# JOP-Lee/READ

Measured on AMD Instinct MI355X. Metric: rendered frames/sec @1216x352, 30M pts, higher is better.
Workload: dtype f32 (matrix-core products from two f16 pieces per operand, three piece pairs, fp32 accumulation)

## Files before the change

### read_amd/csrc/conv.hip

```cpp
#include <limits.h>

#include "common.h"
#include "internal.h"

using namespace readhip;

typedef float floatx16 __attribute__((ext_vector_type(16)));

namespace {

constexpr long long OOB_LIMIT = 0x7ffffff0ll;

struct SrcDev {
    const float *p;
    int C, H, W;
    int sl, sr;
};

struct ConvKArgs {
    SrcDev src[READ_CONV_MAX_SRC];
    const float *mul;
    const float *wp;
    const float *wp_wino;
    const float *wp_w16;
// ... 2341 lines not shown
#pragma unroll
            for (int px = 0; px < 4; ++px) {
                const bool in = (oy + 2 * py < a.outH) & (ox + px < a.outW) & (c0 < a.Cout);
                const int pix = (oy + 2 * py) * a.outW + ox + px;
                rvoff[px] = in ? (unsigned)((pix * a.Cout + c0) * 4) : OOR;
                ovoff[px] = in ? (unsigned)((pix * a.out_cstride + c0) * 4) : OOR;
            }
            f32x4 rv[4];
#pragma unroll
            for (int px = 0; px < 4; ++px) {
                rv[px] = f32x4{0.f, 0.f, 0.f, 0.f};
                if (a.residual) rv[px] = __builtin_bit_cast(f32x4, __builtin_amdgcn_raw_buffer_load_b128(res_rsrc, rvoff[px], 0, 0));
            }
            f32x4 Y[2][4];
#pragma unroll
            for (int h = 0; h < 2; ++h) {
                f32x4 m[6];
#pragma unroll
                for (int fq = 0; fq < 6; ++fq)
#pragma unroll
                    for (int k = 0; k < 4; ++k) asm volatile("v_accvgpr_read_b32 %0, %1" : "=v"(m[fq][k]) : "a"(acc[py + 2 * h][fq][k]));
                at6(m, Y[h]);
                __builtin_amdgcn_sched_barrier(0);
            }
#pragma unroll
            for (int px = 0; px < 4; ++px) {
                f32x4 yf, ym;
                fm_swap(Y[0][px], Y[1][px], yf, ym);
                f32x4 f = __builtin_elementwise_fma(yf, isf, bf);
                const f32x4 mm = __builtin_elementwise_fma(ym, ism, bml);
                if (a.elu) {
                    const f32x4 fe = f * LOG2E;
                    f32x4 e;
#pragma unroll
                    for (int k = 0; k < 4; ++k) e[k] = __builtin_amdgcn_exp2f(fe[k]);
                    e = e + f32x4{-1.0f, -1.0f, -1.0f, -1.0f};
#pragma unroll
                    for (int k = 0; k < 4; ++k) f[k] = f[k] > 0.0f ? f[k] : e[k];
                }
                f32x4 sg_, t;
#pragma unroll
                for (int k = 0; k < 4; ++k) t[k] = __builtin_amdgcn_exp2f(mm[k]);
                t = t + f32x4{1.0f, 1.0f, 1.0f, 1.0f};
#pragma unroll
                for (int k = 0; k < 4; ++k) sg_[k] = __builtin_amdgcn_rcpf(t[k]);
                const f32x4 v = (f * sg_) * sc + sh + rv[px];
                __builtin_amdgcn_raw_buffer_store_b128(__builtin_bit_cast(u32x4, v), out_rsrc, ovoff[px], 0, 0);
                __builtin_amdgcn_sched_barrier(0);
            }
        }
        step_tile(a, by, bx);
        advance();
        gload_patch();
    }
}

struct D3hGeom {
    static constexpr int IH = 10, IW = 34, NPIX = IH * IW;
    static constexpr int XBUF = NPIX * 32;
    static constexpr int NE = NPIX * 8, NI = (NE + 511) / 512;
};

template <bool MUL>
__global__ __launch_bounds__(512, 1) void gated_conv_d3h_kernel(const ConvKArgs a)
{
    using DG = D3hGeom;
    __shared__ __attribute__((aligned(16))) unsigned lds[2 * DG::XBUF];
    __shared__ __attribute__((aligned(16))) float epar[6][32];
    const int tid = threadIdx.x, lane = tid & 63;
    const int wv = __builtin_amdgcn_readfirstlane(tid >> 6), rh = wv & 1, pq = wv >> 1;
    const SrcDev s = a.src[0];
    const int groups = a.CoutPad >> 5, G = gridDim.x;
    const int g = blockIdx.x % groups;
    const int n = a.nchunks;
    constexpr unsigned OOR = 0x80000000u;

    int by = (blockIdx.x / groups) / a.tiles_x, bx = (blockIdx.x / groups) % a.tiles_x;
    int pby = by, pbx = bx, pu = blockIdx.x, pchunk = 0;

    int soff[DG::NI];
    unsigned rel[DG::NI], aoff[DG::NI];
#pragma unroll
    for (int i = 0; i < DG::NI; ++i) {
        const int e = tid + i * 512, pix = e >> 3, q4 = e & 7, ppx = pix % DG::IW;
        soff[i] = pix * 32 + ((((q4 >> 1)) ^ (ppx & 7)) << 2) + ((q4 & 1) << 1);
        rel[i] = (unsigned)(((pix / DG::IW) * s.W + ppx) * s.C + 4 * q4) * 4u;
    }
    const unsigned src_bytes = (unsigned)(a.inH * s.W * s.C) * 4u;
    const auto rsrc = __builtin_amdgcn_make_buffer_rsrc(const_cast<float *>(s.p), 0, src_bytes, 0x00020000);
    const auto rsrc_mul = __builtin_amdgcn_make_buffer_rsrc(const_cast<float *>(MUL ? a.mul : s.p), 0, src_bytes, 0x00020000);
    auto set_patch = [&]() {
        const int y0 = pby * 8 - 1, x0 = pbx * 32 - 1;
        const unsigned base = (unsigned)((y0 * s.W + x0) * s.C) * 4u;
#pragma unroll
        for (int i = 0; i < DG::NI; ++i) {
            const int e = tid + i * 512, pix = e >> 3, ppy = pix / DG::IW, ppx = pix % DG::IW;
            const bool ok = (e < DG::NE) & (ppy >= -y0) & (ppy < a.inH - y0) & (ppx >= -x0) & (ppx < a.inW - x0);
            aoff[i] = ok ? base + rel[i] : OOR;
        }
    };
    auto advance = [&]() {
        if (cursor_advance(a, n, G, pchunk, pu, pby, pbx)) set_patch();
    };
    float4 st[DG::NI], stm[MUL ? DG::NI : 1];
    auto gload = [&]() {
#pragma unroll
// ... 1017 lines not shown
    CFGNM(3, 1, 16, 2, 1, 2, 2, 2, 1),
    CFG(3, 1, 8, 2, 1, 4, 1, 2),
    CFG(3, 1, 8, 1, 1, 4, 1, 2),
    CFG(1, 1, 16, 2, 1, 4, 1, 1),
    CFG(1, 1, 16, 1, 1, 4, 1, 1),
    CFG(1, 1, 16, 2, 2, 2, 2, 1),
    CFG(1, 1, 32, 2, 1, 4, 1, 1),
    CFG(1, 1, 32, 1, 1, 4, 1, 1),
    CFG(1, 1, 32, 2, 2, 2, 2, 1),
    CFG(1, 1, 8, 2, 1, 4, 1, 0),
    CFG(1, 1, 8, 1, 1, 4, 1, 0),
    CFG(3, 2, 16, 1, 1, 4, 1, 1),
    CFG(3, 2, 16, 1, 2, 2, 2, 1),
    CFG(3, 2, 16, 1, 2, 4, 1, 1),
    CFGW(3, 1, 16, 2, 1, 1, 2),
    CFGW(3, 1, 16, 2, 1, 2, 2),
    CFGW(3, 1, 16, 1, 1, 2, 3),
    CFGW(1, 1, 16, 2, 1, 1, 2),
    CFGW(1, 1, 16, 1, 1, 1, 4),
    CFGW(1, 1, 32, 2, 1, 1, 2),
    CFGW(1, 1, 32, 1, 1, 1, 4),
    CFGW(3, 1, 8, 2, 1, 2, 2),
    {"k3s1c16_p1q1_wino", 3, 1, 16, 1, 1, 4, 1, 1, 2, gated_conv_wino_kernel<false, false>, gated_conv_wino_kernel<false, true>, 0, 0, 1},
    CFG(4, 2, 16, 1, 1, 1, 1, 1),
    CFG(4, 2, 16, 1, 1, 4, 1, 1),
    CFG(4, 2, 16, 1, 2, 2, 2, 1),
};
constexpr int N_CONFIGS = sizeof(g_configs) / sizeof(g_configs[0]);

int find_config(int ks, int s, int kc, int P, int QG, int WM, int WN, int PF, int NB)
{
    for (int i = 0; i < N_CONFIGS; ++i) {
        const ConvConfig &c = g_configs[i];
        if (c.KS == ks && c.S == s && c.KC == kc && c.P == P && c.QG == QG && c.WM == WM && c.WN == WN && c.PF == PF &&
            c.NB == NB)
            return i;
    }
    return -1;
}

enum ConvForce {
    CFG_AUTO = -1,
    CFG_PX = -2,
    CFG_W16 = -3,
    CFG_W4 = -5,
    CFG_SC = -6,
    CFG_W4H = -7,
    CFG_D3H = -8,
    CFG_D3H_S2 = -9,
    CFG_PXH = -10,
    CFG_T3H = -11,
    CFG_F4X1 = -12,
    CFG_F4X1_PAIR = -13,
};

int g_prefer_wave = 1;
int g_wino_wgs = 2;
int g_conv_px = 1;
int g_kc32 = 1;
int g_use_wino = 1 << 30;
int g_w4_grid = 0;
int g_w4 = 32;
int g_w4h = 32;
int g_f4x1 = 32;
int g_d3h = 0;
int g_d3h_fam = 32;
int g_d3h_s2 = 32;
int g_pxh = 16;
int g_t3h = 8;
int g_sc = 8;
int g_w16 = 0;
int g_stagger_ticks = 0;

int find_wave_config(int ks, int s, int kc, int P, int QG)
{
    int best = -1;
    for (int i = 0; i < N_CONFIGS; ++i) {
        const ConvConfig &c = g_configs[i];
        if (c.wave && c.KS == ks && c.S == s && c.KC == kc && c.P == P && c.QG == QG) best = i;
    }
    return best;
}

int first_fit(int ks, int s, int kc, int groups, bool tiled_only = false, bool with_mul = false)
{
    for (int i = 0; i < N_CONFIGS; ++i) {
        const ConvConfig &k = g_configs[i];
        if (k.KS == ks && k.S == s && k.KC == kc && groups % (k.WN * k.QG) == 0 && !(tiled_only && (k.wave || k.wino)) && !(with_mul && !k.fn_mul)) return i;
    }
    return -1;
}

int pick_config(int ks, int s, int kc, int groups, int outH, int outW)
{
    const long pixels = (long)outH * outW;
    int c = -1;
    if (ks == 3 && s == 1 && kc == 16) {
        if (groups % 4 == 0 && groups % 8 != 0) c = find_config(3, 1, 16, 2, 2, 2, 2, 1, 2);
        else if (g_prefer_wave) c = find_wave_config(3, 1, 16, 1, 1);
        else if (groups % 8 == 0) c = find_config(3, 1, 16, 2, 1, 2, 2, 2, 1);
        else c = find_config(3, 1, 16, 1, 1, 4, 1, 2, 1);
    } else if (ks == 3 && s == 1 && kc == 8) {
        c = (g_prefer_wave && pixels > 30000) ? find_wave_config(3, 1, 8, 2, 1) : find_config(3, 1, 8, 1, 1, 4, 1, 2, 2);
    } else if (ks == 1 && s == 1 && kc == 32) {
        const long wgs4 = (long)ceil_div(outW, 32) * ceil_div(outH, 4) * (groups / 4);
        if (groups % 4 == 0 && wgs4 >= 128) c = find_config(1, 1, 32, 2, 2, 2, 2, 1, 2);
// ... 64 lines not shown
    {"conv_w4h", &g_w4h, TN_CLAMP, 0, INT_MAX},
    {"conv_f4x1", &g_f4x1, TN_CLAMP, 0, INT_MAX},
    {"conv_d3h", &g_d3h, TN_CLAMP, 0, INT_MAX},
    {"conv_d3h_fam", &g_d3h_fam, TN_CLAMP, 0, INT_MAX},
    {"conv_d3h_s2", &g_d3h_s2, TN_CLAMP, 0, INT_MAX},
    {"conv_pxh", &g_pxh, TN_CLAMP, 0, INT_MAX},
    {"conv_t3h", &g_t3h, TN_CLAMP, 0, INT_MAX},
    {"conv_w4_grid", &g_w4_grid, TN_FLAG, 0, 0},
    {"conv_stagger", &g_stagger_ticks, TN_CLAMP, 0, INT_MAX},
    {"conv_wave", &g_prefer_wave, TN_FLAG, 0, 0},
};
constexpr int N_CONV_KNOBS = sizeof(g_knobs) / sizeof(g_knobs[0]);

int conv_set(const char *key, int v) { return tune_set(g_knobs, N_CONV_KNOBS, key, v); }
int conv_get(const char *key, int *value) { return tune_get(g_knobs, N_CONV_KNOBS, key, value); }
const char *conv_key(int i) { return tune_key(g_knobs, N_CONV_KNOBS, i); }

static unsigned long long *g_trace = nullptr;
static size_t g_trace_records = 0;
void conv_set_trace(void *buf, size_t bytes)
{
    g_trace = (unsigned long long *)buf;
    g_trace_records = buf ? bytes / 64 : 0;
}


static int conv_uses_wino(const read_conv_desc *d)
{
    return d->config < 0 && g_use_wino && !d->pre && d->ksize == 3 && d->stride == 1 && d->n_src == 1 &&
           d->src[0].shift == 0 && d->src[0].C % 16 == 0 && d->wpacked_wino && d->src[0].C <= g_use_wino;
}

static int conv_uses_w4(const read_conv_desc *d)
{
    const bool shape = !d->pre && (!d->linear || !d->residual) && d->ksize == 3 && d->stride == 1 && d->n_src == 1 && d->src[0].shift == 0 &&
                       d->src[0].C % 16 == 0 && d->src[0].C >= 32 && (d->Cout % 32 == 0 || (d->linear && d->Cout % 8 == 0)) && !d->fill_pad && d->wpacked_w4 &&
                       d->out_cstride % 4 == 0 &&
                       (long long)d->src[0].srcH * d->src[0].srcW * d->src[0].C * 4 < (1ll << 31) &&
                       (long long)d->inH * d->inW * d->out_cstride * 4 < (1ll << 31);
    return shape && (d->config == CFG_W4 || (d->config == CFG_AUTO && g_w4 > 0 && d->src[0].C >= g_w4));
}

static int conv_w4_shape(const read_conv_desc *d, const void *operand, bool with_threshold = false)
{
    read_conv_desc t = *d;
    if (!with_threshold) t.config = CFG_W4;
    t.wpacked_w4 = reinterpret_cast<const float *>(operand);
    return conv_uses_w4(&t);
}

static int conv_uses_w4h(const read_conv_desc *d)
{
    if (!d->wpacked_w4h || d->linear || d->mul || d->src[0].C % 32 != 0 || d->Cout % 32 != 0) return 0;
    const bool forced = d->config == CFG_W4H || d->config == CFG_F4X1 || d->config == CFG_F4X1_PAIR;
    if (!forced && (d->config != CFG_AUTO || g_w4h <= 0 || d->src[0].C < g_w4h)) return 0;
    return conv_w4_shape(d, d->wpacked_w4h, !forced);
}

static int conv_uses_d3h(const read_conv_desc *d)
{
    if (!d->wpacked_d3h || d->linear || d->src[0].C % 32 != 0 || d->Cout % 32 != 0) return 0;
    const int min_c = d->mul ? g_d3h_fam : g_d3h;
    if (!(d->config == CFG_D3H || (d->config == CFG_AUTO && min_c > 0 && d->src[0].C >= min_c))) return 0;
    return conv_w4_shape(d, d->wpacked_d3h);
}

static int conv_uses_d3h_s2(const read_conv_desc *d)
{
    const bool shape = d->wpacked_d3h && !d->linear && !d->mul && !d->pre && !d->fill_pad && (d->ksize == 3 || d->ksize == 4) && d->stride == 2 && d->n_src == 1 &&
                       d->src[0].shift == 0 && d->src[0].C % 32 == 0 && d->Cout % 32 == 0 && d->out_cstride % 4 == 0 &&
                       (long long)d->src[0].srcH * d->src[0].srcW * d->src[0].C * 4 < (1ll << 31) &&
                       (long long)d->inH * d->inW * d->out_cstride * 4 < (1ll << 31);
    return shape && (d->config == CFG_D3H_S2 || (d->config == CFG_AUTO && g_d3h_s2 > 0 && d->src[0].C >= g_d3h_s2));
}

static int conv_uses_pxh(const read_conv_desc *d)
{
    if (!d->wpacked_d3h || d->ksize != 1 || d->stride != 1 || d->mul || d->fill_pad || d->n_src < 1 || d->n_src > READ_CONV_MAX_SRC) return 0;
    if (d->pre && d->pre_bilinear) return 0;
    int Cin = 0;
    for (int i = 0; i < d->n_src; ++i) {
        if (d->src[i].C < 8 || d->src[i].C % 8 != 0 || (uintptr_t)d->src[i].data % 16 != 0) return 0;
        Cin += d->src[i].C;
    }
    const bool shape = Cin % 16 == 0 && Cin <= 256 && d->Cout % 4 == 0 && d->out_cstride % 4 == 0 && (uintptr_t)d->out % 16 == 0 &&
                       (uintptr_t)d->params % 16 == 0 && (!d->residual || (uintptr_t)d->residual % 16 == 0) &&
                       (!d->pre || ((uintptr_t)d->pre % 16 == 0 && d->pre_cstride % 4 == 0 && d->pre_f_off % 4 == 0 && d->pre_m_off % 4 == 0));
    return shape && (d->config == CFG_PXH || (d->config == CFG_AUTO && g_pxh > 0 && Cin >= g_pxh));
}

static int conv_uses_t3h(const read_conv_desc *d)
{
    if (!d->wpacked_t3h || d->ksize != 3 || d->stride != 1 || d->mul || d->fill_pad || d->pre || d->n_src != 1 || d->src[0].shift != 0) return 0;
    const int C = d->src[0].C;
    const bool shape = (C == 8 || C == 16 || C == 32) && d->Cout % 4 == 0 && d->out_cstride % 4 == 0 && (uintptr_t)d->out % 16 == 0 &&
                       (uintptr_t)d->src[0].data % 16 == 0 && (uintptr_t)d->params % 16 == 0 && (!d->residual || (uintptr_t)d->residual % 16 == 0) &&
                       (long long)d->inH * d->inW * C * 4 < (1ll << 31);
    return shape && (d->config == CFG_T3H || (d->config == CFG_AUTO && g_t3h > 0 && C <= g_t3h && (long long)d->inH * d->inW >= 16384));
}

static int conv_uses_sc(const read_conv_desc *d)
{
    const bool shape = d->ksize == 3 && d->stride == 1 && d->n_src == 1 && d->src[0].shift == 0 && d->src[0].C == 32 && d->Cout >= 1 &&
                       d->Cout <= 4 && !d->linear && !d->residual && !d->pre && !d->mul && d->wpacked_sc &&
                       (d->out_cstride != 4 || (uintptr_t)d->out % 16 == 0) &&
                       (long long)d->src[0].srcH * d->src[0].srcW * d->src[0].C * 4 < (1ll << 31);
    return shape && (d->config == CFG_SC || (d->config == CFG_AUTO && g_sc));
}

static bool conv_sane(const read_conv_desc *d)
{
    return d->n_src >= 1 && d->n_src <= READ_CONV_MAX_SRC && (d->ksize == 1 || d->ksize == 3 || d->ksize == 4) && (d->stride == 1 || d->stride == 2);
}

static int conv_uses_px(const read_conv_desc *d)
{
    if (!conv_sane(d)) return 0;
    int Cin = 0;
    bool px_pick = d->Cout % 32 != 0 || g_conv_px >= 3;
    for (int i = 0; i < d->n_src; ++i) {
        Cin += d->src[i].C;
        px_pick = px_pick || d->src[i].C % 16 != 0;
    }
    const bool fits = d->ksize == 1 && d->stride == 1 && !d->mul && !d->fill_pad && d->Cout % 4 == 0 && d->out_cstride % 4 == 0 &&
                      (uintptr_t)d->out % 16 == 0 && (uintptr_t)d->params % 16 == 0 && Cin / 8 <= 32 &&
                      (!d->residual || (uintptr_t)d->residual % 16 == 0) &&
                      (!d->pre || ((uintptr_t)d->pre % 16 == 0 && d->pre_cstride % 4 == 0 && d->pre_f_off % 4 == 0 && d->pre_m_off % 4 == 0));
    const bool bil = d->pre && d->pre_bilinear;
    return fits && (d->config == CFG_PX || (bil && d->config < 0) || (d->config == CFG_AUTO && g_conv_px && px_pick));
}

struct ConvShape {
    int Cin, kc;
    int outH, outW, CoutPad, groups;
};

static ConvShape conv_shape(const read_conv_desc *d)
{
    ConvShape s;
    s.Cin = 0;
    s.kc = 16;
    bool all32 = d->ksize == 1;
    for (int i = 0; i < d->n_src; ++i) {
        s.Cin += d->src[i].C;
        if (d->src[i].C % 16) s.kc = 8;
        all32 = all32 && d->src[i].C % 32 == 0;
    }
    if (all32 && (d->config >= 0 ? (d->config < N_CONFIGS && g_configs[d->config].KC == 32) : g_kc32 != 0)) s.kc = 32;
    const int pad = (d->ksize - 1) / 2;
    s.outH = (d->inH + 2 * pad - d->ksize) / d->stride + 1;
    s.outW = (d->inW + 2 * pad - d->ksize) / d->stride + 1;
    s.CoutPad = pad32(d->Cout);
    s.groups = s.CoutPad / 32;
    return s;
}

enum ConvKernel { CK_SC, CK_T3H, CK_PXH, CK_PX, CK_D3H_S2, CK_D3H, CK_F4X1, CK_F4X1_PAIR, CK_W4H, CK_W4, CK_TABLE };

struct ConvRoute {
    ConvKernel kernel;
    int cfg;
    bool wino_auto;
    bool w16;
};

static int w4_units(const ConvShape &s) { return ceil_div(s.outW, 32) * ceil_div(s.outH, 8) * s.groups; }

static bool f4x1_pair_auto(int Cin, int n_units, int n_cu) { return n_units > n_cu && (Cin == 32 || Cin == 128); }

static ConvRoute conv_route(const read_conv_desc *d, const void *wp_f4x1)
{
    ConvRoute r = {CK_TABLE, -1, false, false};
    if (conv_uses_sc(d)) r.kernel = CK_SC;
    else if (conv_uses_t3h(d)) r.kernel = CK_T3H;
    else if (conv_uses_pxh(d)) r.kernel = CK_PXH;
    else if (conv_uses_px(d)) r.kernel = CK_PX;
    else if (conv_uses_d3h_s2(d)) r.kernel = CK_D3H_S2;
    else if (conv_uses_d3h(d)) r.kernel = CK_D3H;
    else if (conv_uses_w4h(d)) {
        const bool forced = d->config == CFG_F4X1 || d->config == CFG_F4X1_PAIR;
        const bool f4x1 = wp_f4x1 && (forced || (d->config == CFG_AUTO && g_f4x1 > 0 && d->src[0].C >= g_f4x1));
        const bool pair = f4x1 && (d->config == CFG_F4X1_PAIR ||
                                   (d->config == CFG_AUTO && f4x1_pair_auto(d->src[0].C, w4_units(conv_shape(d)), device_cus())));
        r.kernel = !f4x1 ? CK_W4H : pair ? CK_F4X1_PAIR : CK_F4X1;
    }
    else if (conv_uses_w4(d)) r.kernel = CK_W4;
    else if (conv_sane(d)) {
        const ConvShape s = conv_shape(d);
        r.cfg = d->config;
        r.wino_auto = conv_uses_wino(d);
        for (int i = N_CONFIGS - 1; r.wino_auto && i >= 0; --i)
            if (g_configs[i].wino) r.cfg = i;
        if (d->linear && r.cfg < 0) r.cfg = first_fit(d->ksize, d->stride, s.kc, s.groups, true, d->mul != nullptr);
        if (r.cfg < 0) r.cfg = pick_config(d->ksize, d->stride, s.kc, s.groups, s.outH, s.outW);
        if (d->config < 0 && d->mul && r.cfg >= 0 && !g_configs[r.cfg].fn_mul) {
            const int m = first_fit(d->ksize, d->stride, s.kc, s.groups, false, true);
            if (m >= 0) r.cfg = m;
        }
        const bool mostly_padding = d->Cout <= 8;
        r.w16 = r.cfg >= 0 && r.cfg < N_CONFIGS && g_configs[r.cfg].wino && !d->linear && d->wpacked_w16 &&
                (d->config == CFG_W16 || (d->config < 0 && (g_w16 || mostly_padding)));
    }
    return r;
}

static int route_family(const ConvRoute &r)
{
    static const int family[] = { 1,  8,  7,  0,  6,  6,
                                  5,  5,  5,  4,  0};
    return r.wino_auto ? 2 : family[r.kernel];
}

int conv_family(const read_conv_desc *d) { return route_family(conv_route(d, nullptr)); }

static int conv_prepare(const read_conv_desc *d, const void *wp_f4x1, ConvKArgs &a, ConvShape &s, ConvRoute &r)
{
    READ_CHECK_ARG(d, "read_gated_conv_forward: null descriptor");
    READ_CHECK_ARG(d->n_src >= 1 && d->n_src <= READ_CONV_MAX_SRC, "read_gated_conv_forward: n_src must be 1..%d",
                   READ_CONV_MAX_SRC);
    READ_CHECK_ARG(d->ksize == 1 || d->ksize == 3 || d->ksize == 4, "read_gated_conv_forward: ksize must be 1,3,4");
    READ_CHECK_ARG(d->stride == 1 || d->stride == 2, "read_gated_conv_forward: stride must be 1 or 2");
    READ_CHECK_ARG(d->inH >= 1 && d->inW >= 1 && d->Cout >= 1, "read_gated_conv_forward: bad sizes");
    READ_CHECK_ARG((d->wpacked || d->wpacked_w4 || d->wpacked_w4h || d->wpacked_d3h || d->wpacked_wino || d->wpacked_t3h || wp_f4x1) && d->params && d->out, "read_gated_conv_forward: null weights/params/out");
    READ_CHECK_ARG(d->out_cstride >= (d->linear ? 2 : 1) * d->Cout, "read_gated_conv_forward: out_cstride too small");
    READ_CHECK_ARG(!d->linear || (!d->residual && !d->fill_pad), "read_gated_conv_forward: linear mode takes no residual / fill");
    READ_CHECK_ARG(!d->mul || d->n_src == 1, "read_gated_conv_forward: mul needs a single source");
    READ_CHECK_ARG((uintptr_t)d->wpacked % 16 == 0, "read_gated_conv_forward: packed weights misaligned");
    r = conv_route(d, wp_f4x1);
    s = conv_shape(d);
    {
        const int family = route_family(r);
        const bool cfg_wino = d->config >= 0 && d->config < N_CONFIGS && g_configs[d->config].wino;
        const bool w16_forced = d->config == CFG_W16;
        READ_CHECK_ARG(d->wpacked || family != 0 || cfg_wino || w16_forced,
                       "read_gated_conv_forward: this launch takes a direct kernel and wpacked is NULL (fragment order not packed)");
        READ_CHECK_ARG(!d->wpacked || (!((const void *)d->wpacked == (const void *)d->wpacked_w4 && family != 4 && family != 5 && family != 6 && family != 7 && family != 8) &&
                                       !((const void *)d->wpacked == (const void *)d->wpacked_wino && family != 2 && !cfg_wino)),
                       "read_gated_conv_forward: wpacked aliases Winograd fragments but the launch takes kernel family %d "
                       "(ask read_conv_kernel_family before packing)", family);
        READ_CHECK_ARG(family != 4 || d->wpacked_w4, "read_gated_conv_forward: F(4x4) launch without wpacked_w4");
        READ_CHECK_ARG(family != 2 || d->wpacked_wino, "read_gated_conv_forward: F(2x2) launch without wpacked_wino");
        READ_CHECK_ARG(family != 1 || d->wpacked_sc, "read_gated_conv_forward: small-Cout launch without wpacked_sc");
    }

    memset(&a, 0, sizeof(a));
    for (int i = 0; i < d->n_src; ++i) {
        const read_conv_src &src = d->src[i];
        READ_CHECK_ARG(src.data && (uintptr_t)src.data % 16 == 0, "read_gated_conv_forward: source %d null or misaligned", i);
        READ_CHECK_ARG(src.C >= 8 && src.C % 8 == 0, "read_gated_conv_forward: source %d has C=%d (need a multiple of 8)", i, src.C);
        READ_CHECK_ARG(src.shift >= -4 && src.shift <= 4, "read_gated_conv_forward: shift out of range");
        READ_CHECK_ARG((long long)src.srcH * src.srcW * src.C < (1ll << 31), "read_gated_conv_forward: source too large");
        const int needH = src.shift >= 0 ? ((d->inH - 1) << src.shift) + 1 : ((d->inH - 1) >> -src.shift) + 1;
        const int needW = src.shift >= 0 ? ((d->inW - 1) << src.shift) + 1 : ((d->inW - 1) >> -src.shift) + 1;
        READ_CHECK_ARG(src.srcH >= needH && src.srcW >= needW, "read_gated_conv_forward: source %d (%dx%d) too small for %dx%d at shift %d",
                       i, src.srcH, src.srcW, d->inH, d->inW, src.shift);
        a.src[i] = SrcDev{src.data, src.C, src.srcH, src.srcW, src.shift > 0 ? src.shift : 0, src.shift < 0 ? -src.shift : 0};
    }
    READ_CHECK_ARG(!d->mul || d->src[0].shift == 0, "read_gated_conv_forward: mul needs shift 0");
    a.n_src = d->n_src;
    READ_CHECK_ARG(s.outH >= 1 && s.outW >= 1, "read_gated_conv_forward: empty output");
    READ_CHECK_ARG((long long)s.outH * s.outW * d->out_cstride * 4 < OOB_LIMIT, "read_gated_conv_forward: output too large");
    if (d->pre) {
// ... 95 lines not shown
    a.nchunks = nsteps;
    a.n_units = ceil_div(s.outH * s.outW, 32 * pt);
    const bool fullq = nsteps % 4 == 0;
    bool uni = true;
    for (int i = 0; i < d->n_src; ++i) uni = uni && d->src[i].C % 16 == 0;
    const int shape = gw == 2 ? 0 : pt == 2 ? 1 : 2, vi = taps ? 12 + shape : shape * 4 + (fullq ? 2 : 0) + (uni ? 1 : 0);
    static const conv_fn fns[15] = {
        gated_conv_pxh_kernel<1, 2, false, 0>, gated_conv_pxh_kernel<1, 2, false, 1>, gated_conv_pxh_kernel<1, 2, true, 0>, gated_conv_pxh_kernel<1, 2, true, 1>,
        gated_conv_pxh_kernel<2, 1, false, 0>, gated_conv_pxh_kernel<2, 1, false, 1>, gated_conv_pxh_kernel<2, 1, true, 0>, gated_conv_pxh_kernel<2, 1, true, 1>,
        gated_conv_pxh_kernel<1, 1, false, 0>, gated_conv_pxh_kernel<1, 1, false, 1>, gated_conv_pxh_kernel<1, 1, true, 0>, gated_conv_pxh_kernel<1, 1, true, 1>,
        gated_conv_pxh_kernel<1, 2, false, 2>, gated_conv_pxh_kernel<2, 1, false, 2>, gated_conv_pxh_kernel<1, 1, false, 2>};
    static bool attr_set_h[15] = {false, false, false, false, false, false, false, false, false, false, false, false, false, false, false};
    return launch_pixel_lane(fns[vi], attr_set_h[vi], 80 * 1024, n_cu * per_cu, gsets, true, lds, stream, a);
}

static int launch_px(ConvKArgs &a, const ConvShape &s, hipStream_t stream)
{
    const int n_cu = device_cus(), nsteps = s.Cin / 8;
    const int gw = (s.groups % 2 == 0 && nsteps <= 16) ? 2 : 1;
    const bool wide = g_conv_px == 2 || g_conv_px == 4;
    const int pt = (gw == 2 ? 1 : 2) * (wide ? 2 : 1);
    const size_t lds = (size_t)nsteps * 2 * gw * 1024;
    int per_cu = (int)((160 * 1024) / (lds + 256));
    const int reg_cap = wide ? 2 : 3;
    per_cu = per_cu < 1 ? 1 : per_cu > reg_cap ? reg_cap : per_cu;
    const int gsets = s.groups / gw;
    a.nchunks = nsteps;
    a.n_units = ceil_div(s.outH * s.outW, 32 * pt);
    const bool fullq = nsteps % 4 == 0;
    static const conv_fn fns[8] = {gated_conv_px_kernel<2, 1>, gated_conv_px_kernel<4, 1>, gated_conv_px_kernel<1, 2>, gated_conv_px_kernel<2, 2>,
                                   gated_conv_px_kernel<2, 1, true>, gated_conv_px_kernel<4, 1, true>, gated_conv_px_kernel<1, 2, true>, gated_conv_px_kernel<2, 2, true>};
    static bool attr_set[8] = {false, false, false, false, false, false, false, false};
    const int vi = (gw == 2 ? 2 : 0) + (wide ? 1 : 0) + (fullq ? 4 : 0);
    return launch_pixel_lane(fns[vi], attr_set[vi], 64 * 1024, n_cu * per_cu, gsets, false, lds, stream, a);
}

static int take_out_gated(const read_conv_desc *d, bool winograd, ConvKArgs &a)
{
    READ_CHECK_ARG(!d->out_gated || (winograd && d->linear && (uintptr_t)d->out_gated % 16 == 0 && d->block_h >= 0 &&
                                     d->valid_h <= d->block_h),
                   "read_gated_conv_forward: out_gated needs a linear launch on the Winograd kernel");
    a.out_gated = d->out_gated;
    a.blk_h = d->block_h;
    a.blk_valid = d->valid_h;
    return READ_OK;
}

static int refuse_f4x1_config(const read_conv_desc *d, bool f4x1)
{
    READ_CHECK_ARG(d->config != CFG_F4X1 || f4x1, "read_gated_conv_forward: config -12 takes the launches of the split-operand 3x3/s1 family "
                   "and needs the F(4,3)-by-rows operand (read_gated_conv_forward_f4x1)");
    READ_CHECK_ARG(d->config != CFG_F4X1_PAIR || f4x1, "read_gated_conv_forward: config -13 takes the launches of the split-operand 3x3/s1 family "
                   "and needs the F(4,3)-by-rows operand (read_gated_conv_forward_f4x1)");
    return READ_OK;
}

static int persistent_grid(ConvKArgs &a, int groups, int cap)
{
    int nwg = a.n_units < cap ? a.n_units : cap;
    nwg -= nwg % groups;
    if (nwg < groups) nwg = groups;
    a.wino_dby = (nwg / groups) / a.tiles_x;
    a.wino_dbx = (nwg / groups) % a.tiles_x;
    return nwg;
}

static int launch_d3h_s2(const read_conv_desc *d, ConvKArgs &a, const ConvShape &s, hipStream_t stream)
{
    const int rc = take_out_gated(d, false, a);
    if (rc != READ_OK) return rc;
    READ_CHECK_ARG((uintptr_t)d->wpacked_d3h % 16 == 0, "read_gated_conv_forward: wpacked_d3h misaligned");
    a.wp_d3h = d->wpacked_d3h;
    a.nchunks = s.Cin / 32;
    a.tiles_x = ceil_div(s.outW, 16);
    const int pairs = (s.CoutPad + 63) / 64;
    a.n_units = a.tiles_x * ceil_div(s.outH, 8) * pairs;
    const int nwg = persistent_grid(a, pairs, device_cus());
    if (d->ksize == 4) hipLaunchKernelGGL((gated_conv_d3h_s2_kernel<4>), dim3((unsigned)nwg), dim3(512), 0, stream, a);
    else hipLaunchKernelGGL((gated_conv_d3h_s2_kernel<3>), dim3((unsigned)nwg), dim3(512), 0, stream, a);
    READ_CHECK_LAUNCH();
    return READ_OK;
}

static int launch_w4_family(const read_conv_desc *d, ConvKArgs &a, const ConvShape &s, ConvKernel kernel, const void *wp_f4x1, hipStream_t stream)
{
    const bool d3h = kernel == CK_D3H, pair = kernel == CK_F4X1_PAIR, f4x1 = pair || kernel == CK_F4X1, w4h = f4x1 || kernel == CK_W4H;
    int rc = take_out_gated(d, kernel == CK_W4, a);
    if (rc != READ_OK) return rc;
    rc = refuse_f4x1_config(d, f4x1);
    if (rc != READ_OK) return rc;
    READ_CHECK_ARG(!w4h || f4x1 || d->wpacked_w4h != wp_f4x1, "read_gated_conv_forward: this launch takes the F(4x4) split-operand kernel "
                   "and only the F(4,3)-by-rows order was packed");
    READ_CHECK_ARG((uintptr_t)(d3h ? d->wpacked_d3h : w4h ? d->wpacked_w4h : (const void *)d->wpacked_w4) % 16 == 0,
                   "read_gated_conv_forward: wpacked_w4 / wpacked_w4h / wpacked_d3h misaligned");
    a.wp_d3h = d->wpacked_d3h;
    READ_CHECK_ARG(!d->mul || (uintptr_t)d->mul % 16 == 0, "read_gated_conv_forward: mul misaligned");
    a.wp_w4h = d->wpacked_w4h;
    a.wp_f4x1 = wp_f4x1;
    READ_CHECK_ARG(!f4x1 || (uintptr_t)wp_f4x1 % 16 == 0, "read_gated_conv_forward: wpacked_f4x1 misaligned");
    a.nchunks = (w4h || d3h) ? s.Cin / 32 : s.Cin / s.kc;
    a.tiles_x = ceil_div(s.outW, 32);
    a.n_units = w4_units(s);
    const int n_cu = (pair ? 2 : 1) * device_cus(), groups = s.groups;
    int cap = n_cu;
    if (g_w4_grid) {
        const int whole = n_cu - n_cu % groups > 0 ? n_cu - n_cu % groups : groups;
        cap = ceil_div(ceil_div(a.n_units, ceil_div(a.n_units, whole)), groups) * groups;
        if (cap > n_cu) cap -= groups;
    }
    const int nwg = persistent_grid(a, groups, cap);
    conv_fn fn = d->linear ? (d->out_gated ? gated_conv_wino4_kernel<false, 1> : gated_conv_wino4_kernel<false, 2>) : d->mul ? gated_conv_wino4_kernel<true> : gated_conv_wino4_kernel<false>;
    unsigned threads = 256;
    if (d3h) {
        fn = d->mul ? gated_conv_d3h_kernel<true> : gated_conv_d3h_kernel<false>;
        threads = 512;
    } else if (pair) fn = f4x1_pair_conv_kernel;
    else if (f4x1) fn = gated_conv_f4x1h_kernel;
    else if (w4h) fn = gated_conv_wino4h_kernel;
    READ_CHECK_ARG(!d->linear || !d->mul, "read_gated_conv_forward: linear launches take no multiplier");
    hipLaunchKernelGGL(fn, dim3((unsigned)nwg), dim3(threads), 0, stream, a);
    READ_CHECK_LAUNCH();
    return READ_OK;
}

static int launch_table(const read_conv_desc *d, ConvKArgs &a, const ConvShape &s, const ConvRoute &r, hipStream_t stream)
{
    const int groups = s.groups;
    READ_CHECK_ARG(!d->linear || d->config < 0 || (d->config < N_CONFIGS && !g_configs[d->config].wave),
                   "read_gated_conv_forward: linear mode needs a workgroup-tiled or Winograd config");
    READ_CHECK_ARG(r.cfg >= 0 && r.cfg < N_CONFIGS, "read_gated_conv_forward: no kernel for k=%d s=%d kc=%d groups=%d",
                   d->ksize, d->stride, s.kc, groups);
    const ConvConfig &c = g_configs[r.cfg];
    READ_CHECK_ARG(c.KS == d->ksize && c.S == d->stride && c.KC == s.kc && groups % (c.WN * c.QG) == 0,
                   "read_gated_conv_forward: config %s does not fit k=%d s=%d kc=%d groups=%d", c.name, d->ksize,
                   d->stride, s.kc, groups);
    a.nchunks = s.Cin / s.kc;
    a.tiles_x = ceil_div(s.outW, 32);
    READ_CHECK_ARG(!d->pre || !c.wino, "read_gated_conv_forward: the Winograd kernel takes no pre-activation addend");
    int rc = take_out_gated(d, c.wino != 0, a);
    if (rc != READ_OK) return rc;
    const int tiles_y = ceil_div(s.outH, c.WM * c.P);
    dim3 grid((unsigned)(a.tiles_x * tiles_y), (unsigned)(groups / (c.WN * c.QG)));
    a.trace = ((size_t)grid.x * grid.y <= g_trace_records) ? g_trace : nullptr;
    if (c.wino) {
        READ_CHECK_ARG(d->wpacked_wino && (uintptr_t)d->wpacked_wino % 16 == 0, "read_gated_conv_forward: config %s needs wpacked_wino", c.name);
        READ_CHECK_ARG(d->n_src == 1 && d->src[0].shift == 0 && d->src[0].C % 16 == 0,
                       "read_gated_conv_forward: the Winograd kernel takes one un-resampled source with C %% 16 == 0");
        a.tiles_x = ceil_div(s.outW, 16);
        a.n_units = a.tiles_x * ceil_div(s.outH, 8) * groups;
        grid = dim3((unsigned)persistent_grid(a, groups, g_wino_wgs * device_cus()), 1);
        a.trace = ((size_t)grid.x * 4 <= g_trace_records) ? g_trace : nullptr;
    }
    if (c.wave) {
        a.tiles_y = ceil_div(s.outH, c.P);
        a.trace = nullptr;
        a.stagger_ticks = g_stagger_ticks;
        a.col_split = a.tiles_x * (groups / c.QG);
        a.n_full = a.col_split * a.tiles_y;
        a.n_units = a.n_full;
        const int want = ceil_div(a.n_units, 4), cap = device_cus() * c.wg_per_cu;
        grid = dim3((unsigned)(want < cap ? want : cap), 1);
    }
    rc = refuse_f4x1_config(d, false);
    if (rc != READ_OK) return rc;
    conv_fn fn = c.fn;
    if (c.wino && a.trace && !d->mul) fn = gated_conv_wino_kernel<true, false>;
    if (d->mul) {
        READ_CHECK_ARG(c.fn_mul, "read_gated_conv_forward: config %s has no multiply variant", c.name);
        READ_CHECK_ARG((uintptr_t)d->mul % 16 == 0, "read_gated_conv_forward: mul misaligned");
        fn = c.fn_mul;
    }
    if (r.w16 && !a.trace) {
        READ_CHECK_ARG((uintptr_t)d->wpacked_w16 % 16 == 0, "read_gated_conv_forward: wpacked_w16 misaligned");
        fn = d->mul ? gated_conv_wino16s_kernel<true> : gated_conv_wino16s_kernel<false>;
    }
    hipLaunchKernelGGL(fn, grid, dim3(256), 0, stream, a);
    READ_CHECK_LAUNCH();
    return READ_OK;
}

int f4x1_pair_occupancy()
{
    int n = 0;
    return hipOccupancyMaxActiveBlocksPerMultiprocessor(&n, f4x1_pair_conv_kernel, 256, 0) == hipSuccess ? n : -1;
}

int launch_gated_conv(const read_conv_desc *d, hipStream_t stream, const void *wp_f4x1)
{
    ConvKArgs a;
    ConvShape s;
    ConvRoute r;
    const int rc = conv_prepare(d, wp_f4x1, a, s, r);
    if (rc != READ_OK) return rc;
    switch (r.kernel) {
    case CK_SC: return launch_sc(d, a, s, stream);
    case CK_T3H:
    case CK_PXH: return launch_pxh(d, a, s, r.kernel == CK_T3H, stream);
    case CK_PX: return launch_px(a, s, stream);
    case CK_D3H_S2: return launch_d3h_s2(d, a, s, stream);
    case CK_D3H:
    case CK_F4X1:
    case CK_F4X1_PAIR:
    case CK_W4H:
    case CK_W4: return launch_w4_family(d, a, s, r.kernel, wp_f4x1, stream);
    case CK_TABLE: return launch_table(d, a, s, r, stream);
    }
    return READ_EINVAL;
}

}

extern "C" int read_conv_f4x1_pair_occupancy(void) { return readhip::f4x1_pair_occupancy(); }

extern "C" int read_conv_kernel_family(const read_conv_desc *desc) { return desc ? readhip::conv_family(desc) : -1; }

extern "C" int read_gated_conv_forward_f4x1(const read_conv_desc *desc, const void *wpacked_f4x1, void *stream)
{
    if (!desc || !wpacked_f4x1 || desc->wpacked_w4h) return readhip::launch_gated_conv(desc, as_stream(stream), wpacked_f4x1);
    read_conv_desc t = *desc;
    t.wpacked_w4h = wpacked_f4x1;
    return readhip::launch_gated_conv(&t, as_stream(stream), wpacked_f4x1);
}

extern "C" int read_gated_conv_forward(const read_conv_desc *desc, void *stream)
{
    return readhip::launch_gated_conv(desc, as_stream(stream), nullptr);
}

namespace {
__global__ __launch_bounds__(256, 1) void mfma_f32_rate_kernel(float *out, int iters)
{
    f32x4 acc[16];
#pragma unroll
    for (int i = 0; i < 16; ++i) acc[i] = f32x4{0.f, 0.f, 0.f, 0.f};
    float a0 = 0.37f + 0.001f * threadIdx.x, b0 = 1.0f - 0.002f * threadIdx.x;
    for (int it = 0; it < iters; ++it) {
#pragma unroll
        for (int m = 0; m < 16; ++m) acc[m] = __builtin_amdgcn_mfma_f32_16x16x4f32(a0, b0, acc[m], 0, 0, 0);
        a0 = a0 * 0.999f + 0.0007f;
        b0 = b0 * 1.0001f - 0.0001f;
    }
    float s = 0.f;
#pragma unroll
    for (int i = 0; i < 16; ++i) s += acc[i][0] + acc[i][3];
    if (s == 1234.5678f) out[blockIdx.x * 256 + threadIdx.x] = s;
}
}

extern "C" int read_mfma_f32_rate_probe(int iters, float *scratch, double *flops, void *stream)
{
    READ_CHECK_ARG(iters > 0 && scratch && flops, "read_mfma_f32_rate_probe: bad arguments");
    int dev = 0, cus = 0;
    if (hipGetDevice(&dev) != hipSuccess || hipDeviceGetAttribute(&cus, hipDeviceAttributeMultiprocessorCount, dev) != hipSuccess || cus < 1) {
        readhip::set_error("read_mfma_f32_rate_probe: cannot query the device");
        return READ_EHIP;
// ... 20 lines not shown
```

Before: 329.7.

## Add 512-thread wide F(4,3) conv kernel covering two output-channel groups

Adds a new persistent F(4,3)-by-rows Winograd conv kernel in which a 512-thread workgroup handles two adjacent 32-channel output groups. The two halves split the input-row transform work, and each half holds its own weight fragments and epilogue parameters. The router picks it automatically for Cin 64/128 when Cout is a multiple of 64 and there are enough units relative to the CU count, and the unit count is halved to match. The aim is better reuse of the staged input tile and better occupancy per CU, in exchange for more LDS and register pressure per workgroup and a new, complex schedule.

```diff
diff --git a/read_amd/csrc/conv.hip b/read_amd/csrc/conv.hip
--- a/read_amd/csrc/conv.hip
+++ b/read_amd/csrc/conv.hip
@@ -2417,6 +2417,237 @@
         step_tile(a, by, bx);
         advance();
         gload_patch();
+    }
+}
+
+__global__ __launch_bounds__(512, 1) void f4x1_wide_conv_kernel(const ConvKArgs a)
+{
+    using WG = F4x1Geom;
+    __shared__ __attribute__((aligned(16))) unsigned lds[WG::LDS_DWORDS];
+    __shared__ __attribute__((aligned(16))) float epar[2][6][32];
+    const int tid = threadIdx.x, lane = tid & 63;
+    const int w8 = __builtin_amdgcn_readfirstlane(tid >> 6), gh = w8 >> 2, wv = w8 & 3;
+    const SrcDev s = a.src[0];
+    const int pairs = a.CoutPad >> 6, G = gridDim.x;
+    const int g = 2 * (blockIdx.x % pairs) + gh;
+    const int n = a.nchunks;
+
+    int by = (blockIdx.x / pairs) / a.tiles_x, bx = (blockIdx.x / pairs) % a.tiles_x;
+    int pby = by, pbx = bx, pu = blockIdx.x, pchunk = 0;
+
+    const int cp = lane & 15, sg = (wv & 1) * 4 + (lane >> 4);
+    const bool third = gh == 0;
+    constexpr unsigned OOR = 0x80000000u;
+    unsigned xoff[6];
+    int rowoff[3];
+    bool rowok[3];
+    const unsigned src_bytes = (unsigned)(a.inH * s.W * s.C) * 4u;
+    const auto rsrc = __builtin_amdgcn_make_buffer_rsrc(const_cast<float *>(s.p), 0, src_bytes, 0x00020000);
+    const auto rsrc_none = __builtin_amdgcn_make_buffer_rsrc(const_cast<float *>(s.p), 0, 0, 0x00020000);
+    auto set_patch = [&]() {
+        int ln;
+        asm volatile("v_mbcnt_lo_u32_b32 %0, -1, 0\n\tv_mbcnt_hi_u32_b32 %0, -1, %0" : "=v"(ln));
+        const int cp = ln & 15, sg = (wv & 1) * 4 + (ln >> 4);
+        const int y0 = pby * 8 - 1 + (wv >> 1) + 6 * gh, x0 = pbx * 32 + 4 * sg - 1;
+#pragma unroll
+        for (int ii = 0; ii < 3; ++ii) {
+            const int yy = y0 + 2 * ii;
+            rowok[ii] = (unsigned)yy < (unsigned)a.inH;
+            const int yc = yy < 0 ? 0 : yy >= a.inH ? a.inH - 1 : yy;
+            rowoff[ii] = yc * s.W * s.C * 4;
+        }
+#pragma unroll
+        for (int c = 0; c < 6; ++c) xoff[c] = (unsigned)(x0 + c) < (unsigned)a.inW ? (unsigned)((x0 + c) * s.C + 2 * cp) * 4u : OOR;
+    };
+    auto advance = [&]() {
+        if (cursor_advance(a, n, G, pchunk, pu, pby, pbx)) set_patch();
+    };
+    f32x2 d2[3][6];
+    auto gload = [&](int ii, int c) {
+        d2[ii][c] = __builtin_bit_cast(f32x2, __builtin_amdgcn_raw_buffer_load_b64(rowok[ii] ? rsrc : rsrc_none, xoff[c], rowoff[ii] + pchunk * 128, 0));
+    };
+    const int vwoff = WG::v_store_off(wv, sg, cp) + 6 * gh * WG::VROW;
+    auto split_store = [&](const f32x2 x, int vb, int ii, int fq) {
+        unsigned hi, lo;
+        split_hl(x.x, x.y, hi, lo);
+        lds[vwoff + vb + 2 * ii * WG::VROW + fq * WG::VFREQ] = hi;
+        lds[vwoff + vb + 2 * ii * WG::VROW + fq * WG::VFREQ + 128] = lo;
+    };
+    auto t_step = [&](int vb, int ii, int j) {
+        if (ii == 2 && !third) return;
+        if (j == 0) bt6(d2[ii][0], d2[ii][1], d2[ii][2], d2[ii][3], d2[ii][4], d2[ii][5]);
+        else split_store(d2[ii][j - 1], vb, ii, j - 1);
+    };
+    auto t_load = [&](int ii) {
+        if (ii == 2 && !third) return;
+#pragma unroll
+        for (int c = 0; c < 6; ++c) gload(ii, c);
+    };
+
+    const auto wrsrc = __builtin_amdgcn_make_buffer_rsrc(const_cast<char *>(WG::w_base(a, g, wv, n)), 0, (unsigned)n * WG::W_BYTES, 0x00020000);
+    const unsigned wvoff = lane * 16;
+    constexpr int RW = 6;
+    u32x4 Wh[RW], Wl[RW];
+    f16x8 Ws;
+    auto wload = [&](int chunk, int fq, int ky) {
+        const int slot = (fq & 1) * 3 + ky;
+        Wh[slot] = __builtin_amdgcn_raw_buffer_load_b128(wrsrc, wvoff, WG::w_frag(chunk, fq, ky), 0);
+        Wl[slot] = __builtin_amdgcn_raw_buffer_load_b128(wrsrc, wvoff, WG::w_frag(chunk, fq, ky) + 1024, 0);
+    };
+    auto wscale = [&](int fq, int ky) {
+        const _Float16 k = (_Float16)0x1p-11f;
+        Ws = __builtin_bit_cast(f16x8, Wh[(fq & 1) * 3 + ky]) * f16x8{k, k, k, k, k, k, k, k};
+    };
+    const int t16 = lane & 15, kl = lane >> 4;
+    const int vrd_e = WG::v_read_off(t16, kl, 0), vrd_o = WG::v_read_off(t16, kl, 1);
+    constexpr int RB = 2, BA = RB - 1;
+    u32x4 Bh[RB], Bl[RB];
+    auto bload = [&](int vb, int idx) {
+        const int fq = idx / 9, sp = idx % 9;
+        const int o = vb + sp * WG::VROW + fq * WG::VFREQ + ((sp & 1) ? vrd_o : vrd_e);
+        Bh[idx % RB] = *reinterpret_cast<const u32x4 *>(__builtin_assume_aligned(lds + o, 16));
+        Bl[idx % RB] = *reinterpret_cast<const u32x4 *>(__builtin_assume_aligned(lds + o + 128, 16));
+    };
+
+    f32x4 acc[4][6];
+    const auto out_rsrc = __builtin_amdgcn_make_buffer_rsrc(a.out, 0, (unsigned)(a.outH * a.outW * a.out_cstride) * 4u, 0x00020000);
+    const auto res_rsrc = __builtin_amdgcn_make_buffer_rsrc(const_cast<float *>(a.residual ? a.residual : a.out), 0,
+                                                            (unsigned)(a.outH * a.outW * a.Cout) * 4u, 0x00020000);
+    epar_load(epar[gh], a, WG::row_scales(a, n), g, tid & 255);
+
+    set_patch();
+#pragma unroll
+    for (int ii = 0; ii < 3; ++ii) t_load(ii);
+#pragma unroll
+    for (int ky = 0; ky < 3; ++ky) wload(0, 0, ky);
+    advance();
+#pragma unroll
+    for (int ii = 0; ii < 3; ++ii) {
+#pragma unroll
+        for (int j = 0; j < 7; ++j) t_step(0, ii, j);
+        t_load(ii);
+    }
+    advance();
+    wscale(0, 0);
+    __syncthreads();
+    bload(0, 0);
+
+    int v_cur = 0, v_nxt = WG::VBUF;
+
+    auto stage_body = [&](int chunk) {
+        int nchunk = chunk + 1;
+        nchunk = nchunk == n ? 0 : nchunk;
+        __builtin_amdgcn_sched_barrier(0);
+#pragma unroll
+        for (int fq = 0; fq < 6; ++fq)
+#pragma unroll
+            for (int sp = 0; sp < 9; ++sp)
+#pragma unroll
+                for (int q = 0; q < 2; ++q) {
+                    const int nb = WG::pair_nb(sp, q), ky = WG::pair_ky(sp, q);
+                    if (!WG::pair_live(sp, q)) continue;
+#pragma unroll
+                    for (int pc = 0; pc < 3; ++pc) {
+                        const int mb = WG::slot_first(sp), ms = WG::slot(sp, q, pc), idx = fq * 9 + sp;
+                        if (ms == mb) {
+                            if (idx == 54 - BA) __syncthreads();
+                            if (idx + BA < 54) bload(v_cur, idx + BA);
+                            else bload(v_nxt, idx + BA - 54);
+                        }
+                        const int ws = (fq & 1) * 3 + ky;
+                        const f16x8 av = pc == 0 ? Ws : __builtin_bit_cast(f16x8, pc == 1 ? Wl[ws] : Wh[ws]);
+                        const f16x8 bv = __builtin_bit_cast(f16x8, pc == 0 ? Bl[idx % RB] : Bh[idx % RB]);
+                        acc[nb][fq] = __builtin_amdgcn_mfma_f32_16x16x32_f16(av, bv, acc[nb][fq], 0, 0, 0);
+                        if (ms == 5 || ms == 11 || ms == 17) {
+                            if (fq < 5) wload(chunk, fq + 1, (ms - 5) / 6);
+                            else wload(nchunk, 0, (ms - 5) / 6);
+                        }
+                        if (pc == 1) {
+                            if (ms < 33) wscale(fq, (ms / 3 + 1) % 3);
+                            else wscale((fq + 1) % 6, 0);
+                        }
+                        if (fq < 3 && (ms & 3) == 2 && ms < 28) t_step(v_nxt, fq, ms >> 2);
+                        if (fq >= 3 && ms == 20) t_load(fq - 3);
+                        __builtin_amdgcn_sched_barrier(0);
+                    }
+                }
+        advance();
+        const int v = v_cur;
+        v_cur = v_nxt;
+        v_nxt = v;
+    };
+
+    for (int u = blockIdx.x; u < a.n_units; u += G) {
+#pragma unroll
+        for (int nb = 0; nb < 4; ++nb)
+#pragma unroll
+            for (int fq = 0; fq < 6; ++fq) asm volatile("v_accvgpr_write_b32 %0, 0\n\tv_accvgpr_write_b32 %1, 0\n\tv_accvgpr_write_b32 %2, 0\n\tv_accvgpr_write_b32 %3, 0"
+                                                        : "=a"(acc[nb][fq][0]), "=a"(acc[nb][fq][1]), "=a"(acc[nb][fq][2]), "=a"(acc[nb][fq][3]));
+        for (int chunk = 0; chunk < n; ++chunk) stage_body(chunk);
+
+        int ln;
+        asm volatile("v_mbcnt_lo_u32_b32 %0, -1, 0\n\tv_mbcnt_hi_u32_b32 %0, -1, %0" : "=v"(ln));
+        const int e16 = ln & 15, cq = (ln >> 4) & 1, hf = ln >> 5;
+        const int c0 = g * 32 + wv * 8 + 4 * cq;
+        const int oy = by * 8 + 4 * hf + (e16 >> 3), ox = bx * 32 + 4 * (e16 & 7);
+        const int cl = wv * 8 + 4 * cq;
+        const auto [bf, bml, sc, sh, isf, ism] = epar_read(epar[gh], cl);
+        constexpr float LOG2E = 1.44269504088896341f;
+        asm volatile("s_nop 15\n\ts_nop 3");
+#pragma unroll
+        for (int py = 0; py < 2; ++py) {
+            unsigned rvoff[4], ovoff[4];
+#pragma unroll
+            for (int px = 0; px < 4; ++px) {
+                const bool in = (oy + 2 * py < a.outH) & (ox + px < a.outW) & (c0 < a.Cout);
+                const int pix = (oy + 2 * py) * a.outW + ox + px;
+                rvoff[px] = in ? (unsigned)((pix * a.Cout + c0) * 4) : OOR;
+                ovoff[px] = in ? (unsigned)((pix * a.out_cstride + c0) * 4) : OOR;
+            }
+            f32x4 rv[4];
+#pragma unroll
+            for (int px = 0; px < 4; ++px) {
+                rv[px] = f32x4{0.f, 0.f, 0.f, 0.f};
+                if (a.residual) rv[px] = __builtin_bit_cast(f32x4, __builtin_amdgcn_raw_buffer_load_b128(res_rsrc, rvoff[px], 0, 0));
+            }
+            f32x4 Y[2][4];
+#pragma unroll
+            for (int h = 0; h < 2; ++h) {
+                f32x4 m[6];
+#pragma unroll
+                for (int fq = 0; fq < 6; ++fq)
+#pragma unroll
+                    for (int k = 0; k < 4; ++k) asm volatile("v_accvgpr_read_b32 %0, %1" : "=v"(m[fq][k]) : "a"(acc[py + 2 * h][fq][k]));
+                at6(m, Y[h]);
+                __builtin_amdgcn_sched_barrier(0);
+            }
+#pragma unroll
+            for (int px = 0; px < 4; ++px) {
+                f32x4 yf, ym;
+                fm_swap(Y[0][px], Y[1][px], yf, ym);
+                f32x4 f = __builtin_elementwise_fma(yf, isf, bf);
+                const f32x4 mm = __builtin_elementwise_fma(ym, ism, bml);
+                if (a.elu) {
+                    const f32x4 fe = f * LOG2E;
+                    f32x4 e;
+#pragma unroll
+                    for (int k = 0; k < 4; ++k) e[k] = __builtin_amdgcn_exp2f(fe[k]);
+                    e = e + f32x4{-1.0f, -1.0f, -1.0f, -1.0f};
+#pragma unroll
+                    for (int k = 0; k < 4; ++k) f[k] = f[k] > 0.0f ? f[k] : e[k];
+                }
+                f32x4 sg_, t;
+#pragma unroll
+                for (int k = 0; k < 4; ++k) t[k] = __builtin_amdgcn_exp2f(mm[k]);
+                t = t + f32x4{1.0f, 1.0f, 1.0f, 1.0f};
+#pragma unroll
+                for (int k = 0; k < 4; ++k) sg_[k] = __builtin_amdgcn_rcpf(t[k]);
+                const f32x4 v = (f * sg_) * sc + sh + rv[px];
+                __builtin_amdgcn_raw_buffer_store_b128(__builtin_bit_cast(u32x4, v), out_rsrc, ovoff[px], 0, 0);
+                __builtin_amdgcn_sched_barrier(0);
+            }
+        }
+        step_tile(a, by, bx);
     }
 }
 
@@ -3540,6 +3771,7 @@
     CFG_T3H = -11,
     CFG_F4X1 = -12,
     CFG_F4X1_PAIR = -13,
+    CFG_F4X1_WIDE = -14,
 };
 
 int g_prefer_wave = 1;
@@ -3710,7 +3942,7 @@
 static int conv_uses_w4h(const read_conv_desc *d)
 {
     if (!d->wpacked_w4h || d->linear || d->mul || d->src[0].C % 32 != 0 || d->Cout % 32 != 0) return 0;
-    const bool forced = d->config == CFG_W4H || d->config == CFG_F4X1 || d->config == CFG_F4X1_PAIR;
+    const bool forced = d->config == CFG_W4H || d->config == CFG_F4X1 || d->config == CFG_F4X1_PAIR || d->config == CFG_F4X1_WIDE;
     if (!forced && (d->config != CFG_AUTO || g_w4h <= 0 || d->src[0].C < g_w4h)) return 0;
     return conv_w4_shape(d, d->wpacked_w4h, !forced);
 }
@@ -3813,7 +4045,7 @@
     return s;
 }
 
-enum ConvKernel { CK_SC, CK_T3H, CK_PXH, CK_PX, CK_D3H_S2, CK_D3H, CK_F4X1, CK_F4X1_PAIR, CK_W4H, CK_W4, CK_TABLE };
+enum ConvKernel { CK_SC, CK_T3H, CK_PXH, CK_PX, CK_D3H_S2, CK_D3H, CK_F4X1, CK_F4X1_PAIR, CK_F4X1_WIDE, CK_W4H, CK_W4, CK_TABLE };
 
 struct ConvRoute {
     ConvKernel kernel;
@@ -3825,6 +4057,8 @@
 static int w4_units(const ConvShape &s) { return ceil_div(s.outW, 32) * ceil_div(s.outH, 8) * s.groups; }
 
 static bool f4x1_pair_auto(int Cin, int n_units, int n_cu) { return n_units > n_cu && (Cin == 32 || Cin == 128); }
+
+static bool f4x1_wide_auto(int Cin, int n_units, int n_cu) { return (Cin == 64 || Cin == 128) && 5 * n_units >= 8 * n_cu; }
 
 static ConvRoute conv_route(const read_conv_desc *d, const void *wp_f4x1)
 {
@@ -3836,11 +4070,14 @@
     else if (conv_uses_d3h_s2(d)) r.kernel = CK_D3H_S2;
     else if (conv_uses_d3h(d)) r.kernel = CK_D3H;
     else if (conv_uses_w4h(d)) {
-        const bool forced = d->config == CFG_F4X1 || d->config == CFG_F4X1_PAIR;
+        const bool wide_fits = d->Cout % 64 == 0;
+        const bool forced = d->config == CFG_F4X1 || d->config == CFG_F4X1_PAIR || (d->config == CFG_F4X1_WIDE && wide_fits);
         const bool f4x1 = wp_f4x1 && (forced || (d->config == CFG_AUTO && g_f4x1 > 0 && d->src[0].C >= g_f4x1));
-        const bool pair = f4x1 && (d->config == CFG_F4X1_PAIR ||
+        const bool wide = f4x1 && wide_fits && (d->config == CFG_F4X1_WIDE ||
+                                   (d->config == CFG_AUTO && f4x1_wide_auto(d->src[0].C, w4_units(conv_shape(d)), device_cus())));
+        const bool pair = f4x1 && !wide && (d->config == CFG_F4X1_PAIR ||
                                    (d->config == CFG_AUTO && f4x1_pair_auto(d->src[0].C, w4_units(conv_shape(d)), device_cus())));
-        r.kernel = !f4x1 ? CK_W4H : pair ? CK_F4X1_PAIR : CK_F4X1;
+        r.kernel = !f4x1 ? CK_W4H : wide ? CK_F4X1_WIDE : pair ? CK_F4X1_PAIR : CK_F4X1;
     }
     else if (conv_uses_w4(d)) r.kernel = CK_W4;
     else if (conv_sane(d)) {
@@ -3865,7 +4102,7 @@
 static int route_family(const ConvRoute &r)
 {
     static const int family[] = { 1,  8,  7,  0,  6,  6,
-                                  5,  5,  5,  4,  0};
+                                  5,  5,  5,  5,  4,  0};
     return r.wino_auto ? 2 : family[r.kernel];
 }
 
@@ -4067,6 +4304,8 @@
                    "and needs the F(4,3)-by-rows operand (read_gated_conv_forward_f4x1)");
     READ_CHECK_ARG(d->config != CFG_F4X1_PAIR || f4x1, "read_gated_conv_forward: config -13 takes the launches of the split-operand 3x3/s1 family "
                    "and needs the F(4,3)-by-rows operand (read_gated_conv_forward_f4x1)");
+    READ_CHECK_ARG(d->config != CFG_F4X1_WIDE || f4x1, "read_gated_conv_forward: config -14 takes the launches of the split-operand 3x3/s1 family "
+                   "and needs the F(4,3)-by-rows operand (read_gated_conv_forward_f4x1)");
     return READ_OK;
 }
 
@@ -4099,7 +4338,7 @@
 
 static int launch_w4_family(const read_conv_desc *d, ConvKArgs &a, const ConvShape &s, ConvKernel kernel, const void *wp_f4x1, hipStream_t stream)
 {
-    const bool d3h = kernel == CK_D3H, pair = kernel == CK_F4X1_PAIR, f4x1 = pair || kernel == CK_F4X1, w4h = f4x1 || kernel == CK_W4H;
+    const bool d3h = kernel == CK_D3H, pair = kernel == CK_F4X1_PAIR, wide = kernel == CK_F4X1_WIDE, f4x1 = pair || wide || kernel == CK_F4X1, w4h = f4x1 || kernel == CK_W4H;
     int rc = take_out_gated(d, kernel == CK_W4, a);
     if (rc != READ_OK) return rc;
     rc = refuse_f4x1_config(d, f4x1);
@@ -4115,8 +4354,8 @@
     READ_CHECK_ARG(!f4x1 || (uintptr_t)wp_f4x1 % 16 == 0, "read_gated_conv_forward: wpacked_f4x1 misaligned");
     a.nchunks = (w4h || d3h) ? s.Cin / 32 : s.Cin / s.kc;
     a.tiles_x = ceil_div(s.outW, 32);
-    a.n_units = w4_units(s);
-    const int n_cu = (pair ? 2 : 1) * device_cus(), groups = s.groups;
+    const int n_cu = (pair ? 2 : 1) * device_cus(), groups = wide ? s.groups / 2 : s.groups;
+    a.n_units = wide ? w4_units(s) / 2 : w4_units(s);
     int cap = n_cu;
     if (g_w4_grid) {
         const int whole = n_cu - n_cu % groups > 0 ? n_cu - n_cu % groups : groups;
@@ -4130,7 +4369,10 @@
         fn = d->mul ? gated_conv_d3h_kernel<true> : gated_conv_d3h_kernel<false>;
         threads = 512;
     } else if (pair) fn = f4x1_pair_conv_kernel;
-    else if (f4x1) fn = gated_conv_f4x1h_kernel;
+    else if (wide) {
+        fn = f4x1_wide_conv_kernel;
+        threads = 512;
+    } else if (f4x1) fn = gated_conv_f4x1h_kernel;
     else if (w4h) fn = gated_conv_wino4h_kernel;
     READ_CHECK_ARG(!d->linear || !d->mul, "read_gated_conv_forward: linear launches take no multiplier");
     hipLaunchKernelGGL(fn, dim3((unsigned)nwg), dim3(threads), 0, stream, a);
@@ -4216,6 +4458,7 @@
     case CK_D3H:
     case CK_F4X1:
     case CK_F4X1_PAIR:
+    case CK_F4X1_WIDE:
     case CK_W4H:
     case CK_W4: return launch_w4_family(d, a, s, r.kernel, wp_f4x1, stream);
     case CK_TABLE: return launch_table(d, a, s, r, stream);
```

New measurement: 339.6, median of 6. 1.03x the previous value.
